# KanaLab/mesh

Hardware: AMD Instinct MI355X
Metric: closest-point queries/sec vs 1M-face mesh at 1/2/4/8 MI355X + HBM GB/s (higher is better)
Workload: dtype f64; 1 GPU; C3: geodesic icosphere freq 224 (1003520 faces, 501762 vertices), 100000000 uniform queries in [-1.1,1.1]^3 (seed 3) per step, sharded contiguously over the GPUs; faces=1003520, queries_total=100000000, queries_per_gpu=100000000

## Files before the change

include/meshsearch.h:

```cpp
#ifndef MESHSEARCH_H_
#define MESHSEARCH_H_

#include <stddef.h>
#include <stdint.h>

#ifdef __cplusplus
extern "C" {
#endif

#define MSH_OK 0
#define MSH_EINVAL 1
#define MSH_EDEVICE 2
#define MSH_ENOMEM 3

#define MSH_NO_FACE 0xFFFFFFFFu

typedef struct msh_tree msh_tree;

typedef struct msh_tree_info {
    int device;
    int kind;
    uint64_t n_points;
    uint64_t n_faces;
    uint64_t n_main_faces;
// ... 27 lines not shown
int msh_device_plan(uint64_t S, int G, uint64_t* begins);

int msh_tree_build(const double* v, size_t P, const uint32_t* f, size_t T, msh_tree** out);
int msh_tree_build_ex(const double* v, size_t P, const uint32_t* f, size_t T, const double* ev, size_t EP,
                      const uint32_t* ef, size_t ET, msh_tree** out);
void msh_tree_free(msh_tree* tree);
int msh_tree_get_info(const msh_tree* tree, msh_tree_info* info);

int msh_tree_nearest(msh_tree* tree, const double* q, size_t S, uint32_t* face, uint32_t* part, double* pt);
int msh_tree_nearest_device(msh_tree* tree, const double* d_q, size_t S, uint32_t* d_face, uint32_t* d_part,
                            double* d_pt, void* stream);
int msh_tree_nearest_stats(msh_tree* tree, const double* d_q, size_t S, uint64_t* nodes, uint64_t* leaves);
int msh_tree_nearest_bary(msh_tree* tree, const double* q, size_t S, uint32_t* face, double* pt, double* w);
int msh_tree_nearest_bary_device(msh_tree* tree, const double* d_q, size_t S, uint32_t* d_face, double* d_pt,
                                 double* d_w, void* stream);

int msh_tree_points_from_faces_device(msh_tree* tree, const double* d_q, size_t S, const uint32_t* d_face,
                                      uint32_t* d_part, double* d_pt, void* stream);

int msh_tree_query_order(msh_tree* tree, const double* d_q, size_t S, uint32_t* d_perm, void* stream);

int msh_tree_set_entry_cut(msh_tree* tree, int G);
int msh_tree_entry_cut_info(const msh_tree* tree, int* state, int* G, uint64_t* bytes, double* build_ms);

int msh_tree_nearest_alongnormal(msh_tree* tree, const double* p, const double* n, size_t S, double* dist,
                                 uint32_t* face, double* pt);
int msh_tree_nearest_alongnormal_device(msh_tree* tree, const double* d_p, const double* d_n, size_t S,
                                        double* d_dist, uint32_t* d_face, double* d_pt, void* stream);
int msh_tree_nearest_alongnormal_stats(msh_tree* tree, const double* d_p, const double* d_n, size_t S, uint64_t* nodes,
                                       uint64_t* leaves);
int msh_visibility_stats(msh_tree* tree, const double* d_cams, size_t C, double min_dist, uint64_t* nodes,
                         uint64_t* leaves);

int msh_tree_intersections(msh_tree* tree, const double* qv, size_t Pq, const uint32_t* qf, size_t Tq, uint32_t* out,
                           size_t* K);

int msh_ntree_build(const double* v, size_t P, const uint32_t* f, size_t T, double eps, msh_tree** out);
int msh_ntree_nearest(msh_tree* tree, const double* q, const double* n, size_t S, uint32_t* face, double* pt);
int msh_ntree_selfintersects(msh_tree* tree, int64_t* count);

int msh_visibility(msh_tree* tree, const double* cams, size_t C, const double* normals, const double* sensors,
                   double min_dist, uint32_t* vis, double* ndc);
int msh_visibility_device(msh_tree* tree, const double* d_cams, size_t C, const double* d_normals,
                          const double* d_sensors, double min_dist, size_t v_begin, size_t v_count, uint32_t* d_vis,
                          double* d_ndc, void* stream);

// ... 52 lines not shown
```

mesh_amd/_native.py:

```python
import ctypes
import os
import threading

import numpy as np

_HERE = os.path.dirname(os.path.abspath(__file__))
LIB_PATH = os.environ.get("MESH_AMD_LIB", os.path.join(_HERE, "lib", "libmeshsearch.so"))

MSH_OK, MSH_EINVAL, MSH_EDEVICE, MSH_ENOMEM = 0, 1, 2, 3
NO_FACE = 0xFFFFFFFF

_c_double_p = ctypes.POINTER(ctypes.c_double)
_c_u32_p = ctypes.POINTER(ctypes.c_uint32)
_c_u64_p = ctypes.POINTER(ctypes.c_uint64)
_c_i64_p = ctypes.POINTER(ctypes.c_int64)
_vp = ctypes.c_void_p
_sz = ctypes.c_size_t
_i = ctypes.c_int

_lib = None
_lock = threading.Lock()

SIGNATURES = [
    ("msh_last_error", ctypes.c_char_p, []),
    ("msh_version", _i, []),
    ("msh_build_id", ctypes.c_char_p, []),
    ("msh_device_count", _i, [ctypes.POINTER(_i)]),
    ("msh_set_device", _i, [_i]),
    ("msh_set_devices", _i, [_i]),
    ("msh_set_device_list", _i, [ctypes.POINTER(_i), _i]),
    ("msh_tree_devices", _i, [_vp, ctypes.POINTER(_i), _i, ctypes.POINTER(_i)]),
    ("msh_device_plan", _i, [ctypes.c_uint64, _i, _c_u64_p]),
    ("msh_tree_build", _i, [_c_double_p, _sz, _c_u32_p, _sz, ctypes.POINTER(_vp)]),
    ("msh_tree_build_ex", _i, [_c_double_p, _sz, _c_u32_p, _sz, _c_double_p, _sz, _c_u32_p, _sz, ctypes.POINTER(_vp)]),
    ("msh_tree_free", None, [_vp]),
    ("msh_tree_get_info", _i, [_vp, _vp]),
    ("msh_tree_nearest", _i, [_vp, _c_double_p, _sz, _c_u32_p, _c_u32_p, _c_double_p]),
    ("msh_tree_nearest_device", _i, [_vp, _vp, _sz, _vp, _vp, _vp, _vp]),
    ("msh_tree_nearest_stats", _i, [_vp, _vp, _sz, _c_u64_p, _c_u64_p]),
    ("msh_tree_nearest_bary", _i, [_vp, _c_double_p, _sz, _c_u32_p, _c_double_p, _c_double_p]),
    ("msh_tree_nearest_bary_device", _i, [_vp, _vp, _sz, _vp, _vp, _vp, _vp]),
    ("msh_tree_points_from_faces_device", _i, [_vp, _vp, _sz, _vp, _vp, _vp, _vp]),
    ("msh_tree_set_entry_cut", _i, [_vp, _i]),
    ("msh_tree_query_order", _i, [_vp, _vp, _sz, _vp, _vp]),
    ("msh_tree_entry_cut_info", _i, [_vp, ctypes.POINTER(_i), ctypes.POINTER(_i), _c_u64_p, ctypes.POINTER(ctypes.c_double)]),
    ("msh_tree_nearest_alongnormal", _i, [_vp, _c_double_p, _c_double_p, _sz, _c_double_p, _c_u32_p, _c_double_p]),
    ("msh_tree_nearest_alongnormal_device", _i, [_vp, _vp, _vp, _sz, _vp, _vp, _vp, _vp]),
    ("msh_tree_nearest_alongnormal_stats", _i, [_vp, _vp, _vp, _sz, _c_u64_p, _c_u64_p]),
    ("msh_visibility_stats", _i, [_vp, _vp, _sz, ctypes.c_double, _c_u64_p, _c_u64_p]),
    ("msh_tree_intersections", _i, [_vp, _c_double_p, _sz, _c_u32_p, _sz, _c_u32_p, ctypes.POINTER(_sz)]),
    ("msh_ntree_build", _i, [_c_double_p, _sz, _c_u32_p, _sz, ctypes.c_double, ctypes.POINTER(_vp)]),
    ("msh_ntree_nearest", _i, [_vp, _c_double_p, _c_double_p, _sz, _c_u32_p, _c_double_p]),
    ("msh_ntree_selfintersects", _i, [_vp, _c_i64_p]),
    ("msh_visibility", _i, [_vp, _c_double_p, _sz, _c_double_p, _c_double_p, ctypes.c_double, _c_u32_p, _c_double_p]),
    ("msh_visibility_device", _i, [_vp, _vp, _sz, _vp, _vp, ctypes.c_double, _sz, _sz, _vp, _vp, _vp]),
    ("msh_vertex_normals", _i, [_c_double_p, _sz, _c_u32_p, _sz, _c_double_p]),
    ("msh_vertex_normals_device", _i, [_vp, _sz, _vp, _sz, _vp, _vp]),
    ("msh_points_build", _i, [_c_double_p, _sz, ctypes.POINTER(_vp)]),
    ("msh_points_nearest", _i, [_vp, _c_double_p, _sz, _c_u32_p, _c_double_p]),
    ("msh_tree_blob_size", _i, [_vp, ctypes.POINTER(_sz)]),
    ("msh_tree_blob_pack", _i, [_vp, _vp, _vp]),
    ("msh_tree_blob_unpack", _i, [_vp, _sz, _i, _vp, ctypes.POINTER(_vp)]),
    ("msh_batch_build", _i, [_c_double_p, _sz, _sz, _c_u32_p, _sz, ctypes.POINTER(_vp)]),
    ("msh_batch_nearest", _i, [_vp, _c_double_p, _sz, _c_u32_p, _c_u32_p, _c_double_p]),
    ("msh_batch_nearest_device", _i, [_vp, _vp, _sz, _vp, _vp, _vp, _vp]),
    ("msh_batch_nearest_bary", _i, [_vp, _c_double_p, _sz, _c_u32_p, _c_double_p, _c_double_p]),
    ("msh_batch_nearest_bary_device", _i, [_vp, _vp, _sz, _vp, _vp, _vp, _vp]),
    ("msh_blob_header_write", _i, [_i, ctypes.c_uint64, ctypes.c_uint64, ctypes.c_uint64, _vp, _sz, _vp]),
# ... 123 lines not shown
            return out
    return [np.empty(shape, dt) for shape, dt in specs]


class Handle(object):

    __slots__ = ("ptr", "kind", "__weakref__")

    def __init__(self, ptr, kind):
        self.ptr = ptr
        self.kind = kind

    def info(self):
        inf = TreeInfo()
        check(lib().msh_tree_get_info(self.ptr, ctypes.byref(inf)))
        return inf

    def set_entry_cut(self, G=-1):
        check(lib().msh_tree_set_entry_cut(self.ptr, int(G)))

    CUT_STATES = {0: "pending", 1: "built", 2: "off", 3: "failed"}

    def entry_cut_info(self):
        st, g, nb, ms = _i(0), _i(0), ctypes.c_uint64(0), ctypes.c_double(0)
        check(lib().msh_tree_entry_cut_info(self.ptr, ctypes.byref(st), ctypes.byref(g), ctypes.byref(nb),
                                            ctypes.byref(ms)))
        return {"state": self.CUT_STATES.get(st.value, st.value), "G": g.value, "bytes": nb.value,
                "build_ms": ms.value}

    def free(self):
        if self.ptr:
            lib().msh_tree_free(self.ptr)
            self.ptr = None

    def __del__(self):
        try:
            self.free()
        except Exception:
            pass

    def __repr__(self):
        return "<meshsearch tree kind=%s at 0x%x>" % (self.kind, self.ptr or 0)


def build_id():
    return lib().msh_build_id().decode()


def source_build_id(extra=""):
    import hashlib
    import os
# ... 119 lines not shown
```

mesh_amd/csrc/api.cpp:

```cpp
#include <hip/hip_runtime.h>

#include <algorithm>
#include <cmath>
#include <cstdarg>
#include <cstdio>
#include <cstdlib>
#include <cstring>
#include <chrono>
#include <map>
#include <atomic>
#include <condition_variable>
#include <functional>
#include <mutex>
#include <set>
#include <string>
#include <thread>
#include <vector>

#include "internal.h"

namespace msh {

static thread_local std::string g_err;
static thread_local int g_device = -1;
// ... 473 lines not shown
    const int G = cut_grid(t, fine);
    double half[3], H = 0.0, lo[3], w[3];
    for (int k = 0; k < 3; ++k) {
        half[k] = 0.5 * ((double)t->scene_hi[k] - (double)t->scene_lo[k]);
        H = std::max(H, half[k]);
    }
    if (!(H > 0.0) || !std::isfinite(H)) {
        set_error("entry cut: degenerate scene box");
        return MSH_EINVAL;
    }
    for (int k = 0; k < 3; ++k) {
        const double m = 0.5 * ((double)t->scene_hi[k] + (double)t->scene_lo[k]);
        const double e = 1.25 * std::max(half[k], 0.05 * H);
        lo[k] = m - e;
        w[k] = 2.0 * e / G;
    }
    const size_t n = (size_t)G * G * G;
    if (n > 0xFFFFFFFFull) {
        set_error("entry cut: %d^3 cells exceed one query call", G);
        return MSH_ENOMEM;
    }
    const bool e4 = t->T <= kEnt4MaxLeaves;
    const size_t rb = cut_rec_bytes(t);
    hipStream_t s = t->stream;
    hipEvent_t e0 = nullptr, e1 = nullptr;
    MSH_HIP(hipEventCreate(&e0));
    hipError_t e = hipEventCreate(&e1);
    if (e != hipSuccess) {
        (void)hipEventDestroy(e0);
        MSH_HIP(e);
    }
    (void)hipEventRecord(e0, s);
    uint32_t* cut = nullptr;
    int st = MSH_OK;
    {
        DevBuf dq, df, dp, dinv, dhint;
        do {
            if ((st = dq.reserve(n * 3 * sizeof(double))) != MSH_OK) break;
            if ((st = df.reserve(n * sizeof(uint32_t))) != MSH_OK) break;
            if ((st = dp.reserve(n * 3 * sizeof(double))) != MSH_OK) break;
            if ((st = dhint.reserve(n * sizeof(int))) != MSH_OK) break;
            if ((st = dinv.reserve(t->T * sizeof(uint32_t))) != MSH_OK) break;
            if ((st = cut_centres(G, lo, w, dq.as<double>(), s)) != MSH_OK) break;
            if ((st = msh_tree_nearest_device(t, dq.as<double>(), n, df.as<uint32_t>(), nullptr, dp.as<double>(), s)) !=
                MSH_OK)
                break;
            if ((st = cut_hints(t, df.as<uint32_t>(), n, dinv.as<uint32_t>(), dhint.as<int>(), s)) != MSH_OK) break;
            dq.release();
            e = dmalloc(&cut, n * rb);
            if (e != hipSuccess) {
                set_error("hipMalloc entry cut (%zu cells): %s", n, hipGetErrorString(e));
                st = MSH_ENOMEM;
                break;
            }
            const uint32_t* half = nullptr;
            if (kCutFromHalf && t->d_cut && 2 * t->cut_G == G && t->cut_wide == (e4 ? 0 : 1) &&
                t->cut_lo[0] == lo[0] && t->cut_lo[1] == lo[1] && t->cut_lo[2] == lo[2])
                half = t->d_cut;
            if ((st = cut_level(t, G, lo, w, dp.as<double>(), dhint.as<int>(), cut, e4, s, half)) != MSH_OK) break;
            (void)hipEventRecord(e1, s);
            if ((e = hipStreamSynchronize(s)) != hipSuccess) {
                set_error("entry cut build: %s", hipGetErrorString(e));
                st = MSH_EDEVICE;
            }
        } while (0);
        (void)hipStreamSynchronize(s);
    }
    if (st == MSH_OK) {
        float ms = 0.f;
        (void)hipEventElapsedTime(&ms, e0, e1);
        t->cut_ms = ms;
        t->d_cut = cut;
        t->cut_wide = e4 ? 0 : 1;
        t->cut_G = G;
        for (int k = 0; k < 3; ++k) {
            t->cut_lo[k] = lo[k];
            t->cut_iw[k] = 1.0 / w[k];
        }
    } else if (cut) {
        (void)dfree(cut);
    }
    (void)hipEventDestroy(e0);
    (void)hipEventDestroy(e1);
    return st;
}

constexpr size_t kCutAutoCellsPerRow = 16;
static void ensure_entry_cut(msh_tree* t, size_t S) {
    if (t->cut_state == kCutOff || t->cut_state == kCutFailed) return;
    if (!cut_applies(t)) {
        if (t->cut_state == kCutPending) t->cut_state = kCutOff;
        return;
    }
    const bool automatic = !t->cut_force && t->cut_req < 0;
// ... 5 lines not shown
        if (t->cut_state == kCutBuilt) {
            if (t->cut_fine || t->cut_rows < fine_rows) return;
        } else if (t->cut_rows < coarse_rows) {
            return;
        }
        fine = t->cut_rows >= fine_rows;
    } else if (t->cut_state == kCutBuilt) {
        return;
    }
    const std::string keep = g_err;
    double staged_ms = 0.0;
    if (kCutStaged && fine && !t->d_cut && t->cut_req < 0) {
        t->cut_state = kCutOff;
        if (build_entry_cut(t, false) == MSH_OK) {
            staged_ms = t->cut_ms;
        } else {
            (void)hipGetLastError();
            t->d_cut = nullptr;
        }
    }
    uint32_t* old = t->d_cut;
    const int old_G = t->cut_G, old_wide = t->cut_wide;
    const double old_ms = t->cut_ms;
    double old_lo[3], old_iw[3];
    for (int k = 0; k < 3; ++k) {
        old_lo[k] = t->cut_lo[k];
        old_iw[k] = t->cut_iw[k];
    }
    t->cut_state = kCutOff;
    const int st = build_entry_cut(t, fine);
    if (st == MSH_OK) {
        t->cut_ms += staged_ms;
        if (old) {
            if (t->ws_done) (void)hipEventSynchronize(t->ws_done);
            (void)dfree(old);
        }
        t->cut_state = kCutBuilt;
        t->cut_fine = fine;
    } else {
        (void)hipGetLastError();
        if (old) {
            t->d_cut = old;
            t->cut_G = old_G;
            t->cut_wide = old_wide;
            t->cut_ms = old_ms;
            for (int k = 0; k < 3; ++k) {
                t->cut_lo[k] = old_lo[k];
                t->cut_iw[k] = old_iw[k];
            }
            t->cut_state = kCutBuilt;
            t->cut_fine = true;
        } else {
            t->cut_state = automatic && ++t->cut_fails <= 2 ? kCutPending : kCutFailed;
            t->cut_rows = 0;
        }
    }
    g_err = keep;
}

constexpr int kResplitLog2 = 16;

static int build_triangles(msh_tree* t, const double* v, size_t Pall, const uint32_t* f, size_t T) {
    hipStream_t s = t->stream;
    hipEvent_t e0, e1;
    MSH_HIP(hipEventCreate(&e0));
    MSH_HIP(hipEventCreate(&e1));
    MSH_HIP(dmalloc(&t->d_v, std::max<size_t>(Pall, 1) * 3 * sizeof(double)));
    MSH_HIP(hipMemcpyAsync(t->d_v, v, Pall * 3 * sizeof(double), hipMemcpyHostToDevice, s));
// ... 938 lines not shown
    t->cut_req = want;
    t->cut_state = kCutPending;
    t->cut_force = true;
    return MSH_OK;
}

int msh_tree_entry_cut_info(const msh_tree* t, int* state, int* G, uint64_t* bytes, double* build_ms) {
    if (!t) { set_error("msh_tree_entry_cut_info: null tree handle"); return MSH_EINVAL; }
    const uint64_t n = t->d_cut ? (uint64_t)t->cut_G * t->cut_G * t->cut_G : 0;
    auto shown = [](const msh_tree* h) { return h->cut_state == kCutPending && !cut_applies(h) ? kCutOff : h->cut_state; };
    if (state) {
        *state = shown(t);
        for (const msh_tree* r : t->replicas) {
            const int rs = shown(r);
            if (rs == kCutFailed || (rs == kCutPending && *state != kCutFailed)) *state = rs;
        }
    }
    if (G) *G = t->d_cut ? t->cut_G : 0;
    if (bytes) *bytes = n * (t->cut_wide ? 64 : 32);
    if (build_ms) *build_ms = t->cut_ms;
    return MSH_OK;
}

int msh_tree_get_info(const msh_tree* t, msh_tree_info* info) {
    if (!t || !info) { set_error("null argument"); return MSH_EINVAL; }
    MSH_TRY(finish_pending(const_cast<msh_tree*>(t)));
    info->device = t->device;
    info->kind = t->kind;
    info->n_points = t->P;
    info->n_faces = t->T;
    info->n_main_faces = t->T_main;
    info->n_nodes = t->T > 0 ? t->B * (t->T - 1) : 0;
    info->n_meshes = t->B;
    const size_t leaf = t->kind == kPoints ? sizeof(PtRec) : sizeof(TriRec);
    info->bytes = info->n_nodes * sizeof(BNode) + t->B * t->T * leaf;
    info->eps = t->eps;
    for (int k = 0; k < 3; ++k) {
        info->scene_lo[k] = t->scene_lo[k];
        info->scene_hi[k] = t->scene_hi[k];
    }
    info->build_ms = t->build_ms;
    info->node_bytes = (uint32_t)sizeof(BNode);
    info->leaf_bytes = (uint32_t)leaf;
    info->max_depth = t->max_depth;
    return MSH_OK;
}
// ... 874 lines not shown
```

mesh_amd/csrc/internal.h:

```cpp
#pragma once
#include <hip/hip_runtime.h>
#include <stddef.h>
#include <stdint.h>

#include <string>
#include <vector>

#include "../../include/meshsearch.h"
#include "common.h"

namespace msh {

void set_error(const char* fmt, ...);

#define MSH_HIP(expr)                                                                           \
    do {                                                                                        \
        hipError_t _e = (expr);                                                                 \
        if (_e != hipSuccess) {                                                                 \
            ::msh::set_error("HIP error %s at %s:%d: %s", hipGetErrorName(_e), __FILE__, __LINE__, #expr); \
            return (_e == hipErrorOutOfMemory) ? MSH_ENOMEM : MSH_EDEVICE;                       \
        }                                                                                       \
    } while (0)

#define MSH_TRY(expr)               \
// ... 97 lines not shown
    size_t vshard_v0 = 0, vshard_nv = 0;
    hipStream_t stream = nullptr;
    hipEvent_t ws_done = nullptr;
    void* h_stage[2] = {nullptr, nullptr};
    void* d_stage[3] = {nullptr, nullptr, nullptr};
    size_t stage_bytes = 0;
    size_t hstage_bytes = 0;
    hipStream_t s_up = nullptr, s_down = nullptr;
    hipEvent_t e_up[3] = {nullptr, nullptr, nullptr}, e_run[3] = {nullptr, nullptr, nullptr},
               e_down[3] = {nullptr, nullptr, nullptr};
    double build_ms = 0.0;
    int max_depth = 0;
    uint32_t* d_cut = nullptr;
    int cut_wide = 0;
    uint32_t* d_face_leaf = nullptr;
    int cut_G = 0;
    int cut_req = -1;
    int cut_state = 0;
    bool cut_force = false;
    uint64_t cut_rows = 0;
    int cut_fails = 0;
    bool cut_fine = false;
    double cut_ms = 0.0;
    double cut_lo[3] = {0, 0, 0}, cut_iw[3] = {0, 0, 0};
    msh::Workspace ws;
    std::vector<msh_tree*> replicas;
    bool pending = false;
    std::vector<void*> pend_free;
    msh::Workspace pend_ws;
    hipEvent_t pend_e0 = nullptr, pend_done = nullptr;
};

namespace msh {

int radix_sort_pairs(uint32_t* keys, uint32_t* vals, uint32_t* keys_alt, uint32_t* vals_alt, size_t n, int bits,
                     Workspace& ws, hipStream_t s, int lo_bit = 0, bool* in_alt = nullptr);
int exclusive_scan_u32(uint32_t* data, size_t n, Workspace& ws, hipStream_t s);

int build_lbvh(msh_tree* tree, const double* d_prim_lo, const double* d_prim_hi, size_t T, uint32_t* d_order);
int build_lbvh_batch(msh_tree* tree, const double* d_prim_lo, const double* d_prim_hi, size_t T, uint32_t* d_order);
int tri_bounds_batch(const double* d_v, size_t P, const uint32_t* d_f, size_t B, size_t T, double* d_lo, double* d_hi,
                     hipStream_t s);
int pack_tri_leaves_batch(const double* d_v, size_t P, const uint32_t* d_f, const uint32_t* d_order, size_t B, size_t T,
                          TriRec* d_out, hipStream_t s);
int query_morton_batch(const msh_tree* tree, const double* d_q, size_t n, size_t S, uint32_t* keys, uint32_t* vals,
                       hipStream_t s, size_t mesh0 = 0);
int mesh_keys(const uint32_t* vals, size_t n, size_t per, uint32_t* keys, hipStream_t s);
double half_diagonal(const double* box, const double* origin);
int upload_origin(msh_tree* tree, hipStream_t s);
int resplit_tree(msh_tree* tree, const double* d_v, const uint32_t* d_f, size_t T, uint32_t* d_order, int log2K);
int build_obb(msh_tree* tree, bool triangles, bool defer = false);
int tri_bounds(const double* d_v, const uint32_t* d_f, size_t T, double* d_lo, double* d_hi, hipStream_t s);
int pack_tri_leaves(const double* d_v, const uint32_t* d_f, const uint32_t* d_order, size_t T, uint32_t face_base,
                    TriRec* d_out, hipStream_t s);
int pack_point_leaves(const double* d_v, const uint32_t* d_order, size_t P, PtRec* d_out, hipStream_t s);
int point_bounds(const double* d_v, size_t P, double* d_lo, double* d_hi, hipStream_t s);

int query_morton(const msh_tree* tree, const double* d_q, size_t S, uint32_t* keys, uint32_t* vals, hipStream_t s);
void query_box(const msh_tree* tree, float* lo, float* hi);
int query_sort(const float* lo, const float* hi, const double* d_q, size_t S, int lo_bit, Workspace& ws, hipStream_t s);
int gather_rows(const double* d_a, const double* d_b, const uint32_t* d_perm, size_t S, double* d_as, double* d_bs,
                uint32_t* d_inv, hipStream_t s);
int unpermute_results(const QRes* d_res, const double* d_w, int nw, const uint32_t* d_inv, size_t S, const SlotOut& o,
                      hipStream_t s);
constexpr int kCutK = 7;
constexpr uint32_t kCutEmpty = 0x7FFFFFFFu;
constexpr size_t kEnt4MaxLeaves = (size_t)1 << 20;
int cut_centres(int G, const double* lo, const double* w, double* d_q, hipStream_t s);
int cut_level(const msh_tree* tree, int G, const double* lo, const double* w, const double* d_pts, const int* d_hint,
              uint32_t* d_rec, bool e4, hipStream_t s, const uint32_t* d_half = nullptr);
int face_leaf_map(const msh_tree* tree, uint32_t* d_inv, hipStream_t s);
int points_from_faces(const msh_tree* tree, const uint32_t* d_inv, const double* d_q, size_t S, const uint32_t* d_face,
                      uint32_t* d_part, double* d_pt, hipStream_t s);
int cut_hints(const msh_tree* tree, const uint32_t* d_face, size_t n, uint32_t* d_inv, int* d_hint, hipStream_t s);
int launch_nearest(const msh_tree* tree, const QueryOrder& ord, size_t S, const SlotOut& o, hipStream_t s);
int launch_nearest_batch(const msh_tree* tree, const QueryOrder& ord, size_t n, size_t S, const SlotOut& o,
                         hipStream_t s, size_t mesh0 = 0);
int launch_nearest_stats(const msh_tree* tree, const QueryOrder& ord, size_t S, unsigned long long* d_counts,
                         hipStream_t s);
int launch_nnearest(const msh_tree* tree, const QueryOrder& ord, size_t S, const SlotOut& o, hipStream_t s);
int launch_points_nearest(const msh_tree* tree, const QueryOrder& ord, size_t S, const SlotOut& o, hipStream_t s);

int launch_alongnormal(const msh_tree* tree, const QueryOrder& ord, size_t S, const SlotOut& o, hipStream_t s);
int launch_visibility(const msh_tree* tree, const double* d_cams, size_t C, const double* d_normals,
                      const double* d_sensors, double min_dist, size_t v0, size_t nv, uint32_t* d_vis, double* d_ndc,
                      hipStream_t s);

int launch_alongnormal_stats(const msh_tree* tree, const QueryOrder& ord, size_t S, unsigned long long* d_counts,
                             hipStream_t s);
int launch_visibility_stats(const msh_tree* tree, const double* d_cams, size_t C, double min_dist,
                            unsigned long long* d_counts, hipStream_t s);

int launch_tri_intersect(const msh_tree* tree, const TriRec* d_qtris, size_t Tq, int self_mode, uint32_t* d_flags,
// ... 15 lines not shown
```

mesh_amd/csrc/nearest.hip:

```cpp
#include <algorithm>
#include <cstddef>
#include <cstdlib>
#include <cstring>
#include <mutex>
#include <vector>
#include <type_traits>

#include "internal.h"


namespace msh {

struct DeferRec {
    uint32_t slot;
    uint32_t face;
    int32_t leaf;
    uint32_t roff;
    double best;
    uint32_t rcnt;
    uint32_t sbound;
};
static_assert(sizeof(DeferRec) == 32, "DeferRec must be 32 B");

#ifndef MSH_P2_SPLIT
// ... 557 lines not shown
#define MSH_LEAN_STEP 1
#endif
#ifndef MSH_LEAN_STATE
#define MSH_LEAN_STATE 1
#endif

constexpr unsigned kRing = 256;
constexpr size_t kListMaxLeaves = (size_t)1 << 26;
constexpr size_t kLeadMinLeaves = 4096;

#ifndef MSH_KNN_WAVES
#define MSH_KNN_WAVES 4
#endif
#define MSH_KNN_ATTR __attribute__((amdgpu_waves_per_eu(MODE == 1 ? 1 : MSH_KNN_WAVES)))
constexpr size_t kNoCell = ~(size_t)0;
__device__ inline size_t cut_cell(const KnnArgs& a, const D3& q) {
    if (!a.cut) return kNoCell;
    const double G = (double)a.cut_G;
    const double ux = (q.x - a.cut_lo[0]) * a.cut_iw[0], uy = (q.y - a.cut_lo[1]) * a.cut_iw[1],
                 uz = (q.z - a.cut_lo[2]) * a.cut_iw[2];
    if (!(ux >= 0.0 && ux < G && uy >= 0.0 && uy < G && uz >= 0.0 && uz < G)) return kNoCell;
    return ((size_t)(unsigned)uz * (size_t)a.cut_G + (unsigned)uy) * (size_t)a.cut_G + (unsigned)ux;
}
__device__ inline const uint32_t* cut_rec(const KnnArgs& a, size_t cell) {
    return a.cut + cell * (a.cut_wide ? 16 : 8);
}
template <class Pol, class W>
__device__ inline bool cut_start(const KnnArgs& a, size_t cell, const Pol& pol, W& w, typename W::Ent* __restrict__ lds,
                                 uint2* __restrict__ spill) {
    const uint32_t* r = cut_rec(a, cell);
    if (a.cut_wide) {
        const uint4* c = reinterpret_cast<const uint4*>(r);
        uint4 e[4];
#pragma unroll
        for (int j = 0; j < 4; ++j) e[j] = c[j];
        auto put = [&](uint32_t ref, uint32_t sb) {
            if (ref != kCutEmpty) w.push(ref, sb, lds, spill);
        };
#pragma unroll
        for (int j = 3; j >= 1; --j) {
            put(e[j].z, e[j].w);
            put(e[j].x, e[j].y);
        }
        put(e[0].z, e[0].w);
    } else {
        const uint4* c = reinterpret_cast<const uint4*>(r);
// ... 81 lines not shown
#if MSH_TILE_PF
        if (lane == 0) nxt = glo < ghi ? atomicAdd(&a.counters[group * 32], 1u) : ~0u;
#endif
        if constexpr (!kLean)
            if (live && a.inv_w && !a.direct) a.inv_w[a.qperm[i]] = (uint32_t)i;
        auto pol = make_pol<MODE>(a, i, q);
        const bool fin = live && finite3(q);
        auto lean_write = [&]() {
            if constexpr (kLean)
                write_direct<MODE>(static_cast<const TriRec*>(a.leaves), (size_t)MSH_COLD_ARG(perm)[i], q, pol,
                                   MSH_COLD_ARG(out_face), MSH_COLD_ARG(out_part), MSH_COLD_ARG(out_pt),
                                   MSH_COLD_ARG(out_w));
        };
        if (live && !fin) {
            if constexpr (kLean)
                lean_write();
            else if (!STATS || a.res)
                write_result<MODE>(a, i, q, pol);
        }
        int hint_leaf = -1;
        const size_t cell = kList && fin ? cut_cell(a, q) : kNoCell;
        if constexpr (kLean) {
            if (cell != kNoCell) {
                const int lf = (int)a.cut[cell * 8];
                if (lf >= 0) pol.test(lf);
            }
        } else if constexpr (MODE == 0 || MODE == 3) {
            if (kList && a.cut && cell != kNoCell && a.phase != 2) {
                const int lf = (int)cut_rec(a, cell)[0];
                if (STATS) hint_leaf = lf;
                if (lf >= 0) {
                    pol.test(lf);
                    if (STATS) {
                        ++n_leaves;
                        ++n_hinted;
                    }
                }
            } else if (fin && (a.phase == 2 || a.phase == 1)) {
                const int lf = a.phase == 2 ? leader_leaf(a, i, q, kFWin, kLead) : leader_leaf(a, i, q, kLWin * kLead2, kLead2);
                if (STATS) hint_leaf = lf;
#if MSH_FOLLOW_CELL
                const int lc = (kList && a.cut && cell != kNoCell) ? (int)cut_rec(a, cell)[0] : -1;
#pragma nounroll
                for (int j = 0; j < 2; ++j) {
                    const int h = j == 0 ? lf : (lc != lf ? lc : -1);
                    if (h >= 0) {
                        pol.test(h);
                        if (STATS) ++n_leaves;
                    }
                }
                if (STATS && lf >= 0) ++n_hinted;
#else
                if (lf >= 0) {
                    pol.test(lf);
                    if (STATS) {
                        ++n_leaves;
                        ++n_hinted;
                    }
                }
#endif
            }
        }
        if (!kLean && a.T == 1) {
            if (fin) {
                pol.test(0);
// ... 994 lines not shown
    oo.w = nullptr;
    return run_knn<1, false>(const_cast<msh_tree*>(tree), a, ord, oo, 0, s, "nnearest");
}

int launch_points_nearest(const msh_tree* tree, const QueryOrder& ord, size_t S, const SlotOut& o, hipStream_t s) {
    KnnArgs a = tree_args(tree, S);
    SlotOut oo{};
    oo.face = o.face;
    oo.dist = o.dist;
    return run_knn<2, false>(const_cast<msh_tree*>(tree), a, ord, oo, 0, s, "points_nearest");
}

__global__ __launch_bounds__(kBlock) void k_cut_centres(int G, double lx, double ly, double lz, double wx, double wy,
                                                        double wz, double* __restrict__ q) {
    const size_t n = (size_t)G * G * G;
    const size_t cell = (size_t)blockIdx.x * kBlock + threadIdx.x;
    if (cell >= n) return;
    const size_t ix = cell % (size_t)G, iy = (cell / (size_t)G) % (size_t)G, iz = cell / ((size_t)G * G);
    q[3 * cell] = lx + ((double)ix + 0.5) * wx;
    q[3 * cell + 1] = ly + ((double)iy + 0.5) * wy;
    q[3 * cell + 2] = lz + ((double)iz + 0.5) * wz;
}

template <bool E4>
__global__ __launch_bounds__(kBlock) void k_cut_level(const BNode* __restrict__ nodes, const TriRec* __restrict__ tris,
                                                      double ox, double oy, double oz, double tm, int G, double lx,
                                                      double ly, double lz, double wx, double wy, double wz,
                                                      const double* __restrict__ pts, const int* __restrict__ hint,
                                                      uint32_t* __restrict__ rec, const uint32_t* __restrict__ crec) {
    constexpr int kw = E4 ? 8 : 16;
    const size_t gid = (size_t)blockIdx.x * kBlock + threadIdx.x;
    const size_t GB = ((size_t)G + 3) / 4, brick = gid >> 6;
    const unsigned ln = (unsigned)(gid & 63);
    if (brick >= GB * GB * GB) return;
    const size_t ix = (brick % GB) * 4 + (ln & 3), iy = ((brick / GB) % GB) * 4 + ((ln >> 2) & 3),
                 iz = (brick / (GB * GB)) * 4 + (ln >> 4);
    if (ix >= (size_t)G || iy >= (size_t)G || iz >= (size_t)G) return;
    const size_t cell = (iz * G + iy) * G + ix;
    const D3 c = D3{lx + ((double)ix + 0.5) * wx, ly + ((double)iy + 0.5) * wy, lz + ((double)iz + 0.5) * wz};
    const double r = 0.5 * sqrt(wx * wx + wy * wy + wz * wz) * 1.001;
    int ref[kCutK];
    float bd[kCutK];
    int stuck[kCutK];
    const int best_leaf = hint[cell];
    ref[0] = 0;
    bd[0] = -1.f;
    stuck[0] = 0;
    int m = 1;
    const D3 pc = D3{pts[3 * cell], pts[3 * cell + 1], pts[3 * cell + 2]};
    float limf = INFINITY;
    {
        const double R = (sqrt(sqdist(c, pc)) + 2.0 * r) * (1.0 + 1e-6);
        if (R < INFINITY) limf = __double2float_ru(R * R * kSlack);
    }
    if (crec) {
        const size_t Gc = (size_t)G / 2;
        const uint32_t* cr = crec + (((iz >> 1) * Gc + (iy >> 1)) * Gc + (ix >> 1)) * kw;
        m = 0;
        for (int k = 0; k < kCutK; ++k) {
            uint32_t rv, bb;
            if (E4) {
                const uint32_t e = cr[1 + k];
                if (e & 0x80000000u) break;
                rv = (uint32_t)Ent4::ref(e);
                bb = __float_as_uint(Ent4::bound(e));
            } else {
                rv = cr[2 + 2 * k];
                if (rv == kCutEmpty) break;
                bb = cr[3 + 2 * k];
            }
            if (__uint_as_float(bb) > limf) continue;
            const float sb = sqrtf(__uint_as_float(bb)) + (float)r;
            ref[m] = (int)rv;
            bd[m] = sb * sb;
            stuck[m] = 0;
            ++m;
        }
        if (m == 0) {
            ref[0] = 0;
            bd[0] = -1.f;
            m = 1;
        }
    }
    const double o3[3] = {ox, oy, oz};
    const QF qf = make_qf(c, o3, tm);
    if (m > 0 && limf < INFINITY) {
        for (int pass = 0; pass < 256; ++pass) {
            bool changed = false;
            const int m0 = m;
            for (int k = 0; k < m0 && k < m; ++k) {
                if (ref[k] < 0) continue;
                if (stuck[k] && m >= stuck[k]) continue;
                const NodeV nd = load_node(nodes, ref[k]);
                float d0, d1;
                node_child_bounds(nd, qf, d0, d1);
                bd[k] = fmaxf(bd[k], fminf(d0, d1));
                const bool h0 = d0 <= limf, h1 = d1 <= limf;
                const int cnt = (int)h0 + (int)h1;
                if (m - 1 + cnt > kCutK) {
                    stuck[k] = m;
                    continue;
                }
                changed = true;
                if (cnt == 0) {
                    ref[k] = ref[m - 1];
                    bd[k] = bd[m - 1];
                    stuck[k] = stuck[m - 1];
                    --m;
                    continue;
                }
                const int c0 = nd.child(0), c1 = nd.child(1);
                stuck[k] = 0;
                if (h0) {
                    ref[k] = c0;
                    bd[k] = d0;
                    if (h1) {
                        ref[m] = c1;
                        bd[m] = d1;
                        stuck[m] = 0;
                        ++m;
// ... 1 lines not shown
                } else {
                    ref[k] = c1;
                    bd[k] = d1;
                }
            }
            if (!changed || m == 0) break;
        }
    }
    if (m == 0) {
        ref[0] = 0;
        bd[0] = 0.f;
        m = 1;
    }
    for (int k = 1; k < m; ++k)
        for (int j = k; j > 0 && bd[j] < bd[j - 1]; --j) {
            const int tr = ref[j];
            ref[j] = ref[j - 1];
            ref[j - 1] = tr;
            const float tb = bd[j];
            bd[j] = bd[j - 1];
            bd[j - 1] = tb;
        }
    uint32_t* out = rec + cell * kw;
    out[0] = (uint32_t)best_leaf;
    if (!E4) out[1] = limf < INFINITY ? __float_as_uint(__double2float_rd(sqrt((double)limf / kSlack) * (1.0 - 1e-7))) : 0u;
    for (int k = 0; k < kCutK; ++k) {
        uint32_t ev = 0xFFFFFFFFu, rv = kCutEmpty, bb = 0u;
        if (k < m) {
            const double b = bd[k] > 0.f ? (double)bd[k] : 0.0;
            const double sv = sqrt(b) * (1.0 - 1e-5) - r * (1.0 + 1e-5);
            bb = __float_as_uint(sv > 0.0 ? __double2float_rd(sv * sv) : 0.f);
            ev = Ent4::make((uint32_t)ref[k], bb);
            rv = (uint32_t)ref[k];
        }
        if (E4) {
            out[1 + k] = ev;
        } else {
            out[2 + 2 * k] = rv;
            out[3 + 2 * k] = bb;
        }
    }
}

__global__ __launch_bounds__(kBlock) void k_face_leaf(const TriRec* __restrict__ tris, size_t T, uint32_t* __restrict__ inv) {
    const size_t l = (size_t)blockIdx.x * kBlock + threadIdx.x;
    if (l >= T) return;
    D3 x, y, z;
    uint32_t face;
// ... 45 lines not shown
        static_cast<const TriRec*>(tree->d_leaves), d_inv, tree->T, d_q, S, d_face, d_part, d_pt);
    MSH_HIP(hipGetLastError());
    return MSH_OK;
}

int cut_hints(const msh_tree* tree, const uint32_t* d_face, size_t n, uint32_t* d_inv, int* d_hint, hipStream_t s) {
    const size_t T = tree->T;
    k_face_leaf<<<(unsigned)((T + kBlock - 1) / kBlock), kBlock, 0, s>>>(static_cast<const TriRec*>(tree->d_leaves), T,
                                                                          d_inv);
    MSH_HIP(hipGetLastError());
    k_cut_hint<<<(unsigned)((n + kBlock - 1) / kBlock), kBlock, 0, s>>>(d_face, n, T, d_inv, d_hint);
    MSH_HIP(hipGetLastError());
    return MSH_OK;
}

int cut_centres(int G, const double* lo, const double* w, double* d_q, hipStream_t s) {
    const size_t n = (size_t)G * G * G;
    k_cut_centres<<<(unsigned)((n + kBlock - 1) / kBlock), kBlock, 0, s>>>(G, lo[0], lo[1], lo[2], w[0], w[1], w[2], d_q);
    MSH_HIP(hipGetLastError());
    return MSH_OK;
}

int cut_level(const msh_tree* tree, int G, const double* lo, const double* w, const double* d_pts, const int* d_hint,
              uint32_t* d_rec, bool e4, hipStream_t s, const uint32_t* d_half) {
    const size_t GB = ((size_t)G + 3) / 4;
    const unsigned nb = (unsigned)((GB * GB * GB * 64 + kBlock - 1) / kBlock);
    const TriRec* tris = static_cast<const TriRec*>(tree->d_leaves);
    const double tm = tree_margin(tree->half_diag);
    TimedLaunch tl("cut_level", s);
    if (e4)
        k_cut_level<true><<<nb, kBlock, 0, s>>>(tree->d_nodes, tris, tree->origin[0], tree->origin[1], tree->origin[2], tm,
                                               G, lo[0], lo[1], lo[2], w[0], w[1], w[2], d_pts, d_hint, d_rec, d_half);
    else
        k_cut_level<false><<<nb, kBlock, 0, s>>>(tree->d_nodes, tris, tree->origin[0], tree->origin[1], tree->origin[2], tm,
                                                G, lo[0], lo[1], lo[2], w[0], w[1], w[2], d_pts, d_hint, d_rec, d_half);
    MSH_HIP(hipGetLastError());
    return MSH_OK;
}

}
```

mesh_amd/csrc/rays.hip:

```cpp
#include <algorithm>

#include "internal.h"

namespace msh {

__device__ inline double det3(const D3& a, const D3& b, const D3& c) { return vdot(vcross(a, b), c); }

__device__ inline bool coplanar_ray_tri(const D3& p, const D3& d, const D3& a, const D3& b, const D3& c, double& tout) {
    const D3 n = vcross(vsub(b, a), vsub(c, a));
    if (n.x == 0.0 && n.y == 0.0 && n.z == 0.0) return false;
    double tlo = 0.0, thi = INFINITY;
    const D3 v[3] = {a, b, c};
#pragma unroll
    for (int e = 0; e < 3; ++e) {
        const D3& s = v[e];
        const D3& t = v[(e + 1) % 3];
        const D3 et = vsub(t, s);
        const double f0 = vdot(n, vcross(et, vsub(p, s)));
        const double f1 = vdot(n, vcross(et, d));
        if (f1 == 0.0) {
            if (f0 < 0.0) return false;
        } else {
            const double tt = -f0 / f1;
            if (f1 > 0.0) tlo = fmax(tlo, tt);
// ... 559 lines not shown
        const size_t i = (size_t)tile * 64 + lane;
#if MSH_RAY_TILE_PF
        if (lane == 0) nxt = glo < ghi ? atomicAdd(&a.counters[group * 32], 1u) : ~0u;
#endif
        if (MODE == 0) {
            const bool live = i < a.S;
            const size_t r = live && a.perm ? (size_t)a.perm[i] : i;
            const size_t ri = a.lazy ? r : i;
            const D3 p = live ? D3{a.p[3 * ri], a.p[3 * ri + 1], a.p[3 * ri + 2]} : D3{0.0, 0.0, 0.0};
            const D3 n = live ? D3{a.n[3 * ri], a.n[3 * ri + 1], a.n[3 * ri + 2]} : D3{0.0, 0.0, 1.0};
            const D3 dp = ray_dir(p, n), pr = vsub(p, org);
            AlongPol pol{a.tris, p, n, make_rayf(pr, dp, a.M, true), INFINITY, MSH_NO_FACE, -1, INFINITY, INFINITY};
            const bool go = live && finite_d3(p) && finite_d3(dp);
            const uint32_t* rec = nullptr;
            float rho = -1.f;
            if (a.cut && go) {
                const double G = (double)a.cut_G;
                const double ux = (p.x - a.cut_lo[0]) * a.cut_iw[0], uy = (p.y - a.cut_lo[1]) * a.cut_iw[1],
                             uz = (p.z - a.cut_lo[2]) * a.cut_iw[2];
                if (ux >= 0.0 && ux < G && uy >= 0.0 && uy < G && uz >= 0.0 && uz < G) {
                    const unsigned ix = (unsigned)ux, iy = (unsigned)uy, iz = (unsigned)uz;
                    const uint32_t* r = a.cut + (((size_t)iz * a.cut_G + iy) * a.cut_G + ix) * (a.cut_wide ? 16 : 8);
                    const int hint = (int)r[0];
                    if (hint >= 0) {
                        const D3 c = D3{a.cut_lo[0] + ((double)ix + 0.5) / a.cut_iw[0],
                                        a.cut_lo[1] + ((double)iy + 0.5) / a.cut_iw[1],
                                        a.cut_lo[2] + ((double)iz + 0.5) / a.cut_iw[2]};
                        double R;
                        if (a.cut_wide) {
                            R = (double)__uint_as_float(r[1]);
                        } else {
                            D3 ta, tb, tc, o;
                            uint32_t f;
                            int part;
                            load_tri(a.tris, hint, ta, tb, tc, f);
                            R = (sqrt(closest_on_triangle(c, ta, tb, tc, o, part)) + 2.0 * a.cut_r) * (1.0 - 1e-9);
                        }
                        const double rr = (R - sqrt(sqdist(p, c))) * (1.0 - 1e-9);
                        if (rr > 0.0) {
                            rec = r;
                            rho = __double2float_rd(rr);
                            pol.capf = __double2float_ru((double)rho * (double)rho * kSlack);
                            pol.relim();
                        }
                    }
                }
            }
// ... 227 lines not shown
```

Baseline: 2.635 billion queries/s.

## Prune entry-cut node candidates with a directional bound and flag affected cells

When building the per-cell entry cut, each cell now uses the direction from the cell centre to its hint point to drop child boxes that cannot hold the closest point for any query in the cell, beyond the plain distance-ball test. Cells where such pruning happened are flagged, either in the hint word (narrow records) or by a zeroed radius (wide records), so the along-normal ray path ignores them, and a count of flagged cells is exposed through a new API. The goal is shorter candidate lists per cell and therefore fewer nodes visited per nearest query. The cost is more work at build time and a subtle correctness argument behind the pruning bound.

```diff
diff --git a/include/meshsearch.h b/include/meshsearch.h
--- a/include/meshsearch.h
+++ b/include/meshsearch.h
@@ -73,6 +73,7 @@
 
 int msh_tree_set_entry_cut(msh_tree* tree, int G);
 int msh_tree_entry_cut_info(const msh_tree* tree, int* state, int* G, uint64_t* bytes, double* build_ms);
+int msh_tree_entry_cut_flagged(const msh_tree* tree, uint64_t* cells);
 
 int msh_tree_nearest_alongnormal(msh_tree* tree, const double* p, const double* n, size_t S, double* dist,
                                  uint32_t* face, double* pt);
diff --git a/mesh_amd/_native.py b/mesh_amd/_native.py
--- a/mesh_amd/_native.py
+++ b/mesh_amd/_native.py
@@ -44,6 +44,7 @@
     ("msh_tree_set_entry_cut", _i, [_vp, _i]),
     ("msh_tree_query_order", _i, [_vp, _vp, _sz, _vp, _vp]),
     ("msh_tree_entry_cut_info", _i, [_vp, ctypes.POINTER(_i), ctypes.POINTER(_i), _c_u64_p, ctypes.POINTER(ctypes.c_double)]),
+    ("msh_tree_entry_cut_flagged", _i, [_vp, _c_u64_p]),
     ("msh_tree_nearest_alongnormal", _i, [_vp, _c_double_p, _c_double_p, _sz, _c_double_p, _c_u32_p, _c_double_p]),
     ("msh_tree_nearest_alongnormal_device", _i, [_vp, _vp, _vp, _sz, _vp, _vp, _vp, _vp]),
     ("msh_tree_nearest_alongnormal_stats", _i, [_vp, _vp, _vp, _sz, _c_u64_p, _c_u64_p]),
@@ -213,11 +214,14 @@
     CUT_STATES = {0: "pending", 1: "built", 2: "off", 3: "failed"}
 
     def entry_cut_info(self):
-        st, g, nb, ms = _i(0), _i(0), ctypes.c_uint64(0), ctypes.c_double(0)
+        st, g, nb, ms, fl = _i(0), _i(0), ctypes.c_uint64(0), ctypes.c_double(0), ctypes.c_uint64(0)
         check(lib().msh_tree_entry_cut_info(self.ptr, ctypes.byref(st), ctypes.byref(g), ctypes.byref(nb),
                                             ctypes.byref(ms)))
+        flagged = getattr(lib(), "msh_tree_entry_cut_flagged", None)
+        if flagged is not None:
+            check(flagged(self.ptr, ctypes.byref(fl)))
         return {"state": self.CUT_STATES.get(st.value, st.value), "G": g.value, "bytes": nb.value,
-                "build_ms": ms.value}
+                "build_ms": ms.value, "flagged": fl.value}
 
     def free(self):
         if self.ptr:
diff --git a/mesh_amd/csrc/api.cpp b/mesh_amd/csrc/api.cpp
--- a/mesh_amd/csrc/api.cpp
+++ b/mesh_amd/csrc/api.cpp
@@ -519,6 +519,7 @@
     }
     const bool e4 = t->T <= kEnt4MaxLeaves;
     const size_t rb = cut_rec_bytes(t);
+    const bool directional = fine || t->cut_req > 0;
     hipStream_t s = t->stream;
     hipEvent_t e0 = nullptr, e1 = nullptr;
     MSH_HIP(hipEventCreate(&e0));
@@ -529,10 +530,17 @@
     }
     (void)hipEventRecord(e0, s);
     uint32_t* cut = nullptr;
+    uint64_t flagged = 0;
     int st = MSH_OK;
     {
-        DevBuf dq, df, dp, dinv, dhint;
+        DevBuf dq, df, dp, dinv, dhint, dflag;
         do {
+            if ((st = dflag.reserve(sizeof(unsigned long long))) != MSH_OK) break;
+            if ((e = hipMemsetAsync(dflag.ptr, 0, sizeof(unsigned long long), s)) != hipSuccess) {
+                set_error("entry cut: %s", hipGetErrorString(e));
+                st = MSH_EDEVICE;
+                break;
+            }
             if ((st = dq.reserve(n * 3 * sizeof(double))) != MSH_OK) break;
             if ((st = df.reserve(n * sizeof(uint32_t))) != MSH_OK) break;
             if ((st = dp.reserve(n * 3 * sizeof(double))) != MSH_OK) break;
@@ -554,12 +562,17 @@
             if (kCutFromHalf && t->d_cut && 2 * t->cut_G == G && t->cut_wide == (e4 ? 0 : 1) &&
                 t->cut_lo[0] == lo[0] && t->cut_lo[1] == lo[1] && t->cut_lo[2] == lo[2])
                 half = t->d_cut;
-            if ((st = cut_level(t, G, lo, w, dp.as<double>(), dhint.as<int>(), cut, e4, s, half)) != MSH_OK) break;
+            if ((st = cut_level(t, G, lo, w, dp.as<double>(), dhint.as<int>(), cut, e4, s, half,
+                                dflag.as<unsigned long long>(), directional)) != MSH_OK)
+                break;
             (void)hipEventRecord(e1, s);
-            if ((e = hipStreamSynchronize(s)) != hipSuccess) {
+            unsigned long long nflag = 0;
+            if ((e = hipMemcpyAsync(&nflag, dflag.ptr, sizeof(nflag), hipMemcpyDeviceToHost, s)) != hipSuccess ||
+                (e = hipStreamSynchronize(s)) != hipSuccess) {
                 set_error("entry cut build: %s", hipGetErrorString(e));
                 st = MSH_EDEVICE;
             }
+            flagged = nflag;
         } while (0);
         (void)hipStreamSynchronize(s);
     }
@@ -567,6 +580,7 @@
         float ms = 0.f;
         (void)hipEventElapsedTime(&ms, e0, e1);
         t->cut_ms = ms;
+        t->cut_flagged = flagged;
         t->d_cut = cut;
         t->cut_wide = e4 ? 0 : 1;
         t->cut_G = G;
@@ -618,6 +632,7 @@
     uint32_t* old = t->d_cut;
     const int old_G = t->cut_G, old_wide = t->cut_wide;
     const double old_ms = t->cut_ms;
+    const uint64_t old_flagged = t->cut_flagged;
     double old_lo[3], old_iw[3];
     for (int k = 0; k < 3; ++k) {
         old_lo[k] = t->cut_lo[k];
@@ -640,6 +655,7 @@
             t->cut_G = old_G;
             t->cut_wide = old_wide;
             t->cut_ms = old_ms;
+            t->cut_flagged = old_flagged;
             for (int k = 0; k < 3; ++k) {
                 t->cut_lo[k] = old_lo[k];
                 t->cut_iw[k] = old_iw[k];
@@ -1624,6 +1640,12 @@
     return MSH_OK;
 }
 
+int msh_tree_entry_cut_flagged(const msh_tree* t, uint64_t* cells) {
+    if (!t || !cells) { set_error("msh_tree_entry_cut_flagged: null argument"); return MSH_EINVAL; }
+    *cells = t->d_cut ? t->cut_flagged : 0;
+    return MSH_OK;
+}
+
 int msh_tree_get_info(const msh_tree* t, msh_tree_info* info) {
     if (!t || !info) { set_error("null argument"); return MSH_EINVAL; }
     MSH_TRY(finish_pending(const_cast<msh_tree*>(t)));
diff --git a/mesh_amd/csrc/internal.h b/mesh_amd/csrc/internal.h
--- a/mesh_amd/csrc/internal.h
+++ b/mesh_amd/csrc/internal.h
@@ -143,6 +143,7 @@
     int cut_fails = 0;
     bool cut_fine = false;
     double cut_ms = 0.0;
+    uint64_t cut_flagged = 0;
     double cut_lo[3] = {0, 0, 0}, cut_iw[3] = {0, 0, 0};
     msh::Workspace ws;
     std::vector<msh_tree*> replicas;
@@ -187,9 +188,15 @@
 constexpr int kCutK = 7;
 constexpr uint32_t kCutEmpty = 0x7FFFFFFFu;
 constexpr size_t kEnt4MaxLeaves = (size_t)1 << 20;
+#ifndef MSH_CUT_DIRECTIONAL
+#define MSH_CUT_DIRECTIONAL 1
+#endif
+constexpr bool kCutDirectional = MSH_CUT_DIRECTIONAL != 0;
+constexpr uint32_t kCutDirFlag = 0x40000000u;
 int cut_centres(int G, const double* lo, const double* w, double* d_q, hipStream_t s);
 int cut_level(const msh_tree* tree, int G, const double* lo, const double* w, const double* d_pts, const int* d_hint,
-              uint32_t* d_rec, bool e4, hipStream_t s, const uint32_t* d_half = nullptr);
+              uint32_t* d_rec, bool e4, hipStream_t s, const uint32_t* d_half = nullptr,
+              unsigned long long* d_nflag = nullptr, bool directional = true);
 int face_leaf_map(const msh_tree* tree, uint32_t* d_inv, hipStream_t s);
 int points_from_faces(const msh_tree* tree, const uint32_t* d_inv, const double* d_q, size_t S, const uint32_t* d_face,
                       uint32_t* d_part, double* d_pt, hipStream_t s);
diff --git a/mesh_amd/csrc/nearest.hip b/mesh_amd/csrc/nearest.hip
--- a/mesh_amd/csrc/nearest.hip
+++ b/mesh_amd/csrc/nearest.hip
@@ -603,6 +603,7 @@
     if (!(ux >= 0.0 && ux < G && uy >= 0.0 && uy < G && uz >= 0.0 && uz < G)) return kNoCell;
     return ((size_t)(unsigned)uz * (size_t)a.cut_G + (unsigned)uy) * (size_t)a.cut_G + (unsigned)ux;
 }
+__device__ inline int cut_hint_leaf(uint32_t w0) { return (int)w0 < 0 ? -1 : (int)(w0 & ~kCutDirFlag); }
 __device__ inline const uint32_t* cut_rec(const KnnArgs& a, size_t cell) {
     return a.cut + cell * (a.cut_wide ? 16 : 8);
 }
@@ -730,12 +731,12 @@
         const size_t cell = kList && fin ? cut_cell(a, q) : kNoCell;
         if constexpr (kLean) {
             if (cell != kNoCell) {
-                const int lf = (int)a.cut[cell * 8];
+                const int lf = cut_hint_leaf(a.cut[cell * 8]);
                 if (lf >= 0) pol.test(lf);
             }
         } else if constexpr (MODE == 0 || MODE == 3) {
             if (kList && a.cut && cell != kNoCell && a.phase != 2) {
-                const int lf = (int)cut_rec(a, cell)[0];
+                const int lf = cut_hint_leaf(cut_rec(a, cell)[0]);
                 if (STATS) hint_leaf = lf;
                 if (lf >= 0) {
                     pol.test(lf);
@@ -748,7 +749,7 @@
                 const int lf = a.phase == 2 ? leader_leaf(a, i, q, kFWin, kLead) : leader_leaf(a, i, q, kLWin * kLead2, kLead2);
                 if (STATS) hint_leaf = lf;
 #if MSH_FOLLOW_CELL
-                const int lc = (kList && a.cut && cell != kNoCell) ? (int)cut_rec(a, cell)[0] : -1;
+                const int lc = (kList && a.cut && cell != kNoCell) ? cut_hint_leaf(cut_rec(a, cell)[0]) : -1;
 #pragma nounroll
                 for (int j = 0; j < 2; ++j) {
                     const int h = j == 0 ? lf : (lc != lf ? lc : -1);
@@ -1789,12 +1790,50 @@
     q[3 * cell + 2] = lz + ((double)iz + 0.5) * wz;
 }
 
-template <bool E4>
+__device__ inline bool cut_dir_drop(const NodeV& nd, bool& h0, bool& h1, const D3& co, const D3& vp, double dp, double r,
+                                    double r2p, double mag) {
+    float ax[3][3], e0[6], e1[6];
+    nd.frame(ax[0], ax[1], ax[2]);
+    nd.extents(e0, e1);
+    double p[3];
+#pragma unroll
+    for (int k = 0; k < 3; ++k) p[k] = (double)ax[k][0] * co.x + (double)ax[k][1] * co.y + (double)ax[k][2] * co.z;
+    const double kf = 1.0 - 1e-6;
+    bool dropped = false;
+#pragma unroll
+    for (int side = 0; side < 2; ++side) {
+        bool& h = side ? h1 : h0;
+        if (!h) continue;
+        const float* e = side ? e1 : e0;
+        double g[3], d2 = 0.0;
+#pragma unroll
+        for (int k = 0; k < 3; ++k) {
+            const double lo = (double)e[k], hi = (double)e[3 + k];
+            g[k] = p[k] < lo ? p[k] - lo : (p[k] > hi ? p[k] - hi : 0.0);
+            d2 += g[k] * g[k];
+        }
+        const double dB = sqrt(d2);
+        if (!(dB > r * (1.0 + 1e-5))) continue;
+        if (!(kf * dB - dp - r2p > 0.0)) continue;
+        const double inv = 1.0 / dB, ks = kf * inv;
+        const D3 w = D3{ks * ((double)ax[0][0] * g[0] + (double)ax[1][0] * g[1] + (double)ax[2][0] * g[2]) - vp.x,
+                        ks * ((double)ax[0][1] * g[0] + (double)ax[1][1] * g[1] + (double)ax[2][1] * g[2]) - vp.y,
+                        ks * ((double)ax[0][2] * g[0] + (double)ax[1][2] * g[1] + (double)ax[2][2] * g[2]) - vp.z};
+        const double lhs = kf * dB - dp - r * (sqrt(vdot(w, w)) + 4.0 * r * inv) - r2p;
+        if (lhs > 9.094947017729282e-13 * (mag + dB)) {
+            h = false;
+            dropped = true;
+        }
+    }
+    return dropped;
+}
+template <bool E4, bool DIR>
 __global__ __launch_bounds__(kBlock) void k_cut_level(const BNode* __restrict__ nodes, const TriRec* __restrict__ tris,
                                                       double ox, double oy, double oz, double tm, int G, double lx,
                                                       double ly, double lz, double wx, double wy, double wz,
                                                       const double* __restrict__ pts, const int* __restrict__ hint,
-                                                      uint32_t* __restrict__ rec, const uint32_t* __restrict__ crec) {
+                                                      uint32_t* __restrict__ rec, const uint32_t* __restrict__ crec,
+                                                      unsigned long long* __restrict__ nflag) {
     constexpr int kw = E4 ? 8 : 16;
     const size_t gid = (size_t)blockIdx.x * kBlock + threadIdx.x;
     const size_t GB = ((size_t)G + 3) / 4, brick = gid >> 6;
@@ -1816,13 +1855,22 @@
     int m = 1;
     const D3 pc = D3{pts[3 * cell], pts[3 * cell + 1], pts[3 * cell + 2]};
     float limf = INFINITY;
+    const double dp = sqrt(sqdist(c, pc));
     {
-        const double R = (sqrt(sqdist(c, pc)) + 2.0 * r) * (1.0 + 1e-6);
+        const double R = (dp + 2.0 * r) * (1.0 + 1e-6);
         if (R < INFINITY) limf = __double2float_ru(R * R * kSlack);
     }
+    const D3 co = D3{c.x - ox, c.y - oy, c.z - oz};
+    const bool dir = DIR && dp > r * (1.0 + 1e-5) && dp < INFINITY;
+    const float dp2f = __double2float_rd(dp * dp);
+    const D3 vp = D3{(c.x - pc.x) / dp, (c.y - pc.y) / dp, (c.z - pc.z) / dp};
+    const double mag = fabs(co.x) + fabs(co.y) + fabs(co.z) + fabs(pc.x - ox) + fabs(pc.y - oy) + fabs(pc.z - oz) + dp;
+    const double r2p = 2.0 * r * r / dp;
+    bool flagged = false;
     if (crec) {
         const size_t Gc = (size_t)G / 2;
         const uint32_t* cr = crec + (((iz >> 1) * Gc + (iy >> 1)) * Gc + (ix >> 1)) * kw;
+        flagged = E4 ? ((int)cr[0] >= 0 && (cr[0] & kCutDirFlag)) : cr[1] == 0u;
         m = 0;
         for (int k = 0; k < kCutK; ++k) {
             uint32_t rv, bb;
@@ -1862,7 +1910,9 @@
                 float d0, d1;
                 node_child_bounds(nd, qf, d0, d1);
                 bd[k] = fmaxf(bd[k], fminf(d0, d1));
-                const bool h0 = d0 <= limf, h1 = d1 <= limf;
+                bool h0 = d0 <= limf, h1 = d1 <= limf;
+                if (dir && ((h0 && d0 > dp2f) || (h1 && d1 > dp2f)) && cut_dir_drop(nd, h0, h1, co, vp, dp, r, r2p, mag))
+                    flagged = true;
                 const int cnt = (int)h0 + (int)h1;
                 if (m - 1 + cnt > kCutK) {
                     stuck[k] = m;
@@ -1910,8 +1960,15 @@
             bd[j - 1] = tb;
         }
     uint32_t* out = rec + cell * kw;
-    out[0] = (uint32_t)best_leaf;
-    if (!E4) out[1] = limf < INFINITY ? __float_as_uint(__double2float_rd(sqrt((double)limf / kSlack) * (1.0 - 1e-7))) : 0u;
+    out[0] = (uint32_t)best_leaf | (E4 && flagged && best_leaf >= 0 ? kCutDirFlag : 0u);
+    if (!E4)
+        out[1] = limf < INFINITY && !flagged
+                     ? __float_as_uint(__double2float_rd(sqrt((double)limf / kSlack) * (1.0 - 1e-7)))
+                     : 0u;
+    if (nflag) {
+        const unsigned long long fl = __ballot(flagged);
+        if (flagged && (unsigned)__ffsll((long long)fl) - 1u == ln) atomicAdd(nflag, (unsigned long long)__popcll(fl));
+    }
     for (int k = 0; k < kCutK; ++k) {
         uint32_t ev = 0xFFFFFFFFu, rv = kCutEmpty, bb = 0u;
         if (k < m) {
@@ -2003,18 +2060,21 @@
 }
 
 int cut_level(const msh_tree* tree, int G, const double* lo, const double* w, const double* d_pts, const int* d_hint,
-              uint32_t* d_rec, bool e4, hipStream_t s, const uint32_t* d_half) {
+              uint32_t* d_rec, bool e4, hipStream_t s, const uint32_t* d_half, unsigned long long* d_nflag,
+              bool directional) {
     const size_t GB = ((size_t)G + 3) / 4;
     const unsigned nb = (unsigned)((GB * GB * GB * 64 + kBlock - 1) / kBlock);
     const TriRec* tris = static_cast<const TriRec*>(tree->d_leaves);
     const double tm = tree_margin(tree->half_diag);
     TimedLaunch tl("cut_level", s);
-    if (e4)
-        k_cut_level<true><<<nb, kBlock, 0, s>>>(tree->d_nodes, tris, tree->origin[0], tree->origin[1], tree->origin[2], tm,
-                                               G, lo[0], lo[1], lo[2], w[0], w[1], w[2], d_pts, d_hint, d_rec, d_half);
+    auto launch = [&](auto kern) {
+        kern<<<nb, kBlock, 0, s>>>(tree->d_nodes, tris, tree->origin[0], tree->origin[1], tree->origin[2], tm, G, lo[0], lo[1],
+                                   lo[2], w[0], w[1], w[2], d_pts, d_hint, d_rec, d_half, d_nflag);
+    };
+    if (directional && kCutDirectional)
+        e4 ? launch(k_cut_level<true, true>) : launch(k_cut_level<false, true>);
     else
-        k_cut_level<false><<<nb, kBlock, 0, s>>>(tree->d_nodes, tris, tree->origin[0], tree->origin[1], tree->origin[2], tm,
-                                                G, lo[0], lo[1], lo[2], w[0], w[1], w[2], d_pts, d_hint, d_rec, d_half);
+        e4 ? launch(k_cut_level<true, false>) : launch(k_cut_level<false, false>);
     MSH_HIP(hipGetLastError());
     return MSH_OK;
 }
diff --git a/mesh_amd/csrc/rays.hip b/mesh_amd/csrc/rays.hip
--- a/mesh_amd/csrc/rays.hip
+++ b/mesh_amd/csrc/rays.hip
@@ -605,7 +605,7 @@
                     const unsigned ix = (unsigned)ux, iy = (unsigned)uy, iz = (unsigned)uz;
                     const uint32_t* r = a.cut + (((size_t)iz * a.cut_G + iy) * a.cut_G + ix) * (a.cut_wide ? 16 : 8);
                     const int hint = (int)r[0];
-                    if (hint >= 0) {
+                    if (hint >= 0 && !((uint32_t)hint & kCutDirFlag)) {
                         const D3 c = D3{a.cut_lo[0] + ((double)ix + 0.5) / a.cut_iw[0],
                                         a.cut_lo[1] + ((double)iy + 0.5) / a.cut_iw[1],
                                         a.cut_lo[2] + ((double)iz + 0.5) / a.cut_iw[2]};
```

Measured after the change: 2.876 billion queries/s, median of 6. 1.09x the previous value.
